# g8a9/multi-modal-emotion

Hardware: AMD Instinct MI355X
Metric: utterances/sec fwd+bwd (+clip_grad_norm_+AdamW inside the timed step), TAV (BERT+Wav2Vec2+VideoMAE) b=32, 1/2/4/8 MI355X (higher is better)
Workload: dtype bf16; 1 GPU; tav_nn.py TAV preset B (bert 12 L + wav2vec2 12 L / 768 + videomae 12 L / 768 on 16 frames + fusion 12 L), global batch 32 = 32 per GPU x 1, text 128 tok, audio 80000 samples, video 16x3x224x224 (104 fusion / 1464 encoder tokens), 547.0 GFLOP forward per utterance; global_batch=32, per_gpu_batch=32, parallelism=dp1, weights=random init (seeded), no checkpoints offline, launch=hipGraph replay

## Files before the change

multi-modal-emotion_amd/csrc/gemm.hip:

```cpp
#include "common.h"
#include <type_traits>
#include "tavhip_internal.h"
#include "gemm_plan.h"

namespace tav {

struct GemmNT {
    const char* A; const char* B; char* C; char* Cpre; const float* bias; const char* gelu_in; const float* resid;
    int M, N, K;
    long lda, ldb, ldc, ld_pre, ld_gelu, ld_resid;
    int nzg;
    long a_zb, a_zg, b_zb, b_zg, c_zb, c_zg, bias_zg;
    long g_zb;
    int act, accumulate;
    float alpha;
    int tiles_m, tiles_n;
    const float* sa; const float* sb;
};

TAV_DEV int swz(int row, int chunk) { return chunk ^ ((row >> 1) & 7); }

enum { NT_GEN = 0, NT_PLAIN = 1, NT_RESID = 2, NT_GELU_D = 3, NT_MUL_D = 4 };
template <typename T, typename TO, int TM, int NST, int NW, int TNW, int EPI = NT_GEN>
__global__ __launch_bounds__(64 * NW, NW == 4 ? 2 : 1) __attribute__((amdgpu_waves_per_eu(2, 2))) void gemm_nt_kernel(const GemmNT p) {
// ... 79 lines not shown
        for (int t = 0; t < TNW; ++t) fb0[t] = *reinterpret_cast<const uint4*>(cB + off_b[0][t]);
#pragma unroll
        for (int t = 0; t < TM; ++t) fa1[t] = *reinterpret_cast<const uint4*>(cA + off_a[1][t]);
#pragma unroll
        for (int t = 0; t < TNW; ++t) fb1[t] = *reinterpret_cast<const uint4*>(cB + off_b[1][t]);
        __builtin_amdgcn_sched_barrier(0);
#pragma unroll
        for (int tn = 0; tn < TNW; ++tn) {
#pragma unroll
            for (int tm = 0; tm < TM; ++tm) {
                if constexpr (F8) mma16_fp8(fb0[tn], fb1[tn], fa0[tm], fa1[tm], acc[tn][tm]);
                else mma16<T>(fb0[tn], fa0[tm], acc[tn][tm]);
            }
            if constexpr (decltype(prefetch)::value) {
                __builtin_amdgcn_sched_barrier(0);
#pragma unroll
                for (int pc = tn * NP / TNW; pc < (tn + 1) * NP / TNW; ++pc) stage_piece(pc, ko, nxt);
                __builtin_amdgcn_sched_barrier(0);
            }
        }
        if constexpr (!F8) {
#pragma unroll
            for (int tn = 0; tn < TNW; ++tn)
#pragma unroll
                for (int tm = 0; tm < TM; ++tm) mma16<T>(fb1[tn], fa1[tm], acc[tn][tm]);
        }
    };
    auto ktile25 = [&](int kt, int cl, int cs, auto issue_s, auto issue_l) {
        constexpr bool IS = decltype(issue_s)::value, IL = decltype(issue_l)::value;
        if constexpr (IS) asm volatile("s_waitcnt vmcnt(%0)" ::"n"(TM) : "memory");
        else wait_vmcnt0();
        __syncthreads();
        const char* cA = sA + cl * TILE_A;
        const char* cB = sB + cs * TILE_B;
        const int nl = cl == 0 ? 2 : cl - 1;
        const int ns = cs ^ 1;
#pragma unroll
        for (int t = 0; t < TM; ++t) fa0[t] = *reinterpret_cast<const uint4*>(cA + off_a[0][t]);
#pragma unroll
        for (int t = 0; t < TNW; ++t) fb0[t] = *reinterpret_cast<const uint4*>(cB + off_b[0][t]);
#pragma unroll
        for (int t = 0; t < TM; ++t) fa1[t] = *reinterpret_cast<const uint4*>(cA + off_a[1][t]);
#pragma unroll
        for (int t = 0; t < TNW; ++t) fb1[t] = *reinterpret_cast<const uint4*>(cB + off_b[1][t]);
        __builtin_amdgcn_sched_barrier(0);
#pragma unroll
        for (int tn = 0; tn < TNW; ++tn) {
#pragma unroll
            for (int tm = 0; tm < TM; ++tm) mma16<T>(fb0[tn], fa0[tm], acc[tn][tm]);
            if constexpr (IS || IL) {
                __builtin_amdgcn_sched_barrier(0);
                if constexpr (IS) {
                    if (tn < PB) stage_b(tn, (unsigned)(kt + 1) * 128u, ns);
                }
                if constexpr (IL) {
                    if (tn >= PB && tn - PB < TM) stage_a(tn - PB, (unsigned)(kt + 2) * 128u, nl);
                }
                __builtin_amdgcn_sched_barrier(0);
            }
        }
#pragma unroll
        for (int tn = 0; tn < TNW; ++tn)
#pragma unroll
            for (int tm = 0; tm < TM; ++tm) mma16<T>(fb1[tn], fa1[tm], acc[tn][tm]);
    };
    if constexpr (R25) {
        static_assert(!R25 || PB + TM <= TNW, "one DMA piece per MFMA group");
        auto stage_l = [&](unsigned ko, int slot) {
#pragma unroll
            for (int j = 0; j < TM; ++j) stage_a(j, ko, slot);
        };
        auto stage_s = [&](unsigned ko, int slot) {
#pragma unroll
            for (int j = 0; j < PB; ++j) stage_b(j, ko, slot);
        };
        stage_l(0u, 0);
        stage_s(0u, 0);
        if (nk > 1) stage_l(128u, 1);
        int cl = 0, cs = 0, kt = 0;
        for (; kt + 2 < nk; ++kt) { ktile25(kt, cl, cs, std::true_type{}, std::true_type{}); cl = cl == 2 ? 0 : cl + 1; cs ^= 1; }
        if (kt + 1 < nk) { ktile25(kt, cl, cs, std::true_type{}, std::false_type{}); cl = cl == 2 ? 0 : cl + 1; cs ^= 1; ++kt; }
        if (kt < nk) ktile25(kt, cl, cs, std::false_type{}, std::false_type{});
    } else {
#pragma unroll
    for (int t = 0; t < NST - 1; ++t)
        if (t < nk) {
#pragma unroll
            for (int pc = 0; pc < NP; ++pc) stage_piece(pc, (unsigned)t * 128u, t);
        }
    int cur = 0;
    int kt = 0;
    for (; kt + NST - 1 < nk; ++kt) { ktile(kt, cur, std::true_type{}); cur = cur + 1 == NST ? 0 : cur + 1; }
    for (; kt < nk; ++kt) { ktile(kt, cur, std::false_type{}); cur = cur + 1 == NST ? 0 : cur + 1; }
    }

    __syncthreads();
    float* sC = reinterpret_cast<float*>(smem);
    constexpr int ROWB_C = BN * 4;
    constexpr int CPR = BN / 4;
    constexpr int LDS_BYTES = NST * (TILE_A + TILE_B);
    constexpr int EP_ROWS = (LDS_BYTES / ROWB_C) < BM ? (LDS_BYTES / ROWB_C) / (16 * TM) * (16 * TM) : BM;
    constexpr int NPASS = BM / EP_ROWS;
    static_assert(EP_ROWS >= 16 * TM && BM % EP_ROWS == 0, "epilogue staging");
    const long coff = zb * p.c_zb + zg * p.c_zg;
    TO* C = reinterpret_cast<TO*>(p.C) + coff;
    TO* Cpre = p.Cpre ? reinterpret_cast<TO*>(p.Cpre) + coff : nullptr;
    const TS* Gin = p.gelu_in ? reinterpret_cast<const TS*>(p.gelu_in) + (zb * p.g_zb + zg * p.c_zg) : nullptr;
    const float alpha = p.alpha * (p.sa ? *p.sa : 1.f) * (p.sb ? *p.sb : 1.f);
    const float* R = p.resid ? p.resid + coff : nullptr;
    constexpr bool GEN = EPI == NT_GEN;
    const bool f_resid = GEN ? (R != nullptr) : (EPI == NT_RESID);
    const bool f_pre = GEN ? (Cpre != nullptr && !(p.act & 2)) : false;
    const bool f_act3 = GEN ? ((p.act & 3) == 3) : (EPI == NT_GELU_D);
    const bool f_gelu = GEN ? ((p.act & 3) == 1) : false;
    const bool f_gin = GEN ? (Gin != nullptr) : (EPI == NT_MUL_D);
    const bool f_gin_d = GEN ? ((p.act & 4) != 0) : true;
    const bool f_acc = GEN ? (p.accumulate != 0) : false;
    const int ch = tid % CPR, rr = tid / CPR;
    constexpr int RPI = 64 * NW / CPR;
    const int n = n0 + 4 * ch;
    f32x4 bv = {0.f, 0.f, 0.f, 0.f};
    if (n < p.N && p.bias) bv = ld4(p.bias + zg * p.bias_zg + n);
    constexpr int NIT = EP_ROWS / RPI;
    static_assert(EP_ROWS % RPI == 0 && NIT <= 16, "epilogue rows per thread");
    const bool interior = m0 + BM <= p.M && n0 + BN <= p.N;
    constexpr int PD = (EPI == NT_MUL_D) ? NIT : (NIT > 8 ? 8 : NIT);
    constexpr bool EARLY = (TNW == 4);
    const bool pre_r = f_resid, pre_g = !pre_r && f_gin && sizeof(TS) == 2, pre_c = !pre_r && !pre_g && f_acc && sizeof(TO) == 4;
    const bool any_side = pre_r || pre_c || pre_g;
    char* const Cb = reinterpret_cast<char*>(C + (long)m0 * p.ldc);
    char* const Pb = Cpre ? reinterpret_cast<char*>(Cpre + (long)m0 * p.ld_pre) : nullptr;
    const char* const Gb = Gin ? reinterpret_cast<const char*>(Gin + (long)m0 * p.ld_gelu) : nullptr;
    const char* const Rb = R ? reinterpret_cast<const char*>(R + (long)m0 * p.ld_resid) : nullptr;
    const unsigned s_c = RPI * (unsigned)p.ldc * sizeof(TO), s_p = RPI * (unsigned)p.ld_pre * sizeof(TO);
    const unsigned s_g = RPI * (unsigned)p.ld_gelu * sizeof(TS), s_r = RPI * (unsigned)p.ld_resid * 4u;
    auto run_pass = [&](int row_lo, auto full_tag) __attribute__((always_inline)) {
        constexpr bool FULL = decltype(full_tag)::value;
        const unsigned row = (unsigned)(row_lo + rr);
        const unsigned o_c = (row * (unsigned)p.ldc + (unsigned)n) * (unsigned)sizeof(TO), o_p = (row * (unsigned)p.ld_pre + (unsigned)n) * (unsigned)sizeof(TO);
        const unsigned o_g = (row * (unsigned)p.ld_gelu + (unsigned)n) * (unsigned)sizeof(TS), o_r = (row * (unsigned)p.ld_resid + (unsigned)n) * 4u;
        f32x4 side[PD];
        auto side_load = [&](int it) __attribute__((always_inline)) -> f32x4 {
            const int m = m0 + row_lo + rr + it * RPI;
            f32x4 v = {0.f, 0.f, 0.f, 0.f};
            if (FULL || (n < p.N && m < p.M)) {
                if (pre_r) v = ld4(reinterpret_cast<const float*>(Rb + (o_r + it * s_r)));
                else if (pre_c) { if constexpr (sizeof(TO) == 4) v = ld4(reinterpret_cast<const float*>(Cb + (o_c + it * s_c))); }
                else if (pre_g) {
                    const uint2 w = *reinterpret_cast<const uint2*>(Gb + (o_g + it * s_g));
                    v[0] = __uint_as_float(w.x);
                    v[1] = __uint_as_float(w.y);
                }
            }
            return v;
        };
        auto side_loads = [&]() __attribute__((always_inline)) {
            if (!any_side) return;
#pragma unroll
            for (int it = 0; it < PD; ++it) side[it] = side_load(it);
        };
        if constexpr (EARLY) side_loads();
        if (wm * 16 * TM >= row_lo && wm * 16 * TM < row_lo + EP_ROWS) {
#pragma unroll
            for (int tm = 0; tm < TM; ++tm) {
                const int r = wm * 16 * TM + tm * 16 + i - row_lo;
#pragma unroll
                for (int tn = 0; tn < TNW; ++tn) {
                    const int cc = wn * 4 * TNW + tn * 4 + g;
                    *reinterpret_cast<f32x4*>(reinterpret_cast<char*>(sC) + r * ROWB_C + ((cc ^ (r & 31)) << 4)) = acc[tn][tm];
                }
            }
        }
        if constexpr (!EARLY) side_loads();
        __syncthreads();
        if (FULL || n < p.N) {
            auto staged = [&](int it) __attribute__((always_inline)) -> f32x4 {
                const int r = rr + it * RPI;
                return *reinterpret_cast<const f32x4*>(reinterpret_cast<const char*>(sC) + r * ROWB_C + ((ch ^ (r & 31)) << 4));
            };
            f32x4 v_next = staged(0);
#pragma unroll
            for (int it = 0; it < NIT; ++it) {
                const int r = rr + it * RPI;
                const int m = m0 + row_lo + r;
                const f32x4 sv = side[it % PD];
                if constexpr (PD < NIT) { if (it + PD < NIT && any_side) side[it % PD] = side_load(it + PD); }
                f32x4 v = v_next;
                if (it + 1 < NIT) v_next = staged(it + 1);
                if (FULL || m < p.M) {
                    v = v * alpha + bv;
                    if (f_pre) st4(reinterpret_cast<TO*>(Pb + (o_p + it * s_p)), v);
                    if (f_act3) {
                        f32x4 d, y4;
                        gelu_both4_t<TS>(v, y4, d);
                        v = y4;
                        if (GEN ? Cpre != nullptr : true) st4(reinterpret_cast<TO*>(Pb + (o_p + it * s_p)), d);
                    } else if (f_gelu) { v[0] = gelu_t<TS>(v[0]); v[1] = gelu_t<TS>(v[1]); v[2] = gelu_t<TS>(v[2]); v[3] = gelu_t<TS>(v[3]); }
                    if (f_gin) {
                        f32x4 u;
                        if (pre_g) {
                            const uint32_t w0 = __float_as_uint(sv[0]), w1 = __float_as_uint(sv[1]);
                            u = f32x4{bf16_bits_to_f32(w0 & 0xffffu), bf16_bits_to_f32(w0 >> 16), bf16_bits_to_f32(w1 & 0xffffu), bf16_bits_to_f32(w1 >> 16)};
                        }
                        else u = ld4(reinterpret_cast<const TS*>(Gb + (o_g + it * s_g)));
                        if (f_gin_d) v *= u;
                        else { v[0] *= gelu_grad_t<TS>(u[0]); v[1] *= gelu_grad_t<TS>(u[1]); v[2] *= gelu_grad_t<TS>(u[2]); v[3] *= gelu_grad_t<TS>(u[3]); }
                    }
                    if (pre_r) v += sv;
                    if (f_acc) {
                        if (pre_c) v += sv;
                        else v += ld4(reinterpret_cast<const TO*>(Cb + (o_c + it * s_c)));
                    }
                    st4(reinterpret_cast<TO*>(Cb + (o_c + it * s_c)), v);
                }
            }
        }
    };
    if constexpr (GEN) {
#pragma unroll 1
        for (int pass = 0; pass < NPASS; ++pass) {
            if (pass) __syncthreads();
            run_pass(pass * EP_ROWS, std::false_type{});
        }
    } else {
        if (interior) {
#pragma unroll
            for (int pass = 0; pass < NPASS; ++pass) {
                if (pass) __syncthreads();
                run_pass(pass * EP_ROWS, std::true_type{});
            }
        } else {
#pragma unroll
            for (int pass = 0; pass < NPASS; ++pass) {
                if (pass) __syncthreads();
                run_pass(pass * EP_ROWS, std::false_type{});
            }
        }
    }
}

struct GemmTN {
    const char* A; const char* B; float* S;
    float* bias_part;
    int bias_spread;
    int N1, N2;
    long lda, ldb;
    int rows_per_batch;
    long a_zb, b_zb;
    int chunk_rows;
    int chunks_per_batch;
    int tiles_1, tiles_2;
};

template <typename T> struct TNTile {
    static constexpr int ES = ET<T>::ES, ROWB = 128 * ES, CPR = ROWB / 16;
    static TAV_DEV int sw(int row, int chunk) { return ES == 2 ? (chunk ^ ((row & 7) << 1)) : (chunk ^ (((row >> 2) & 1) << 2)); }
};
template <typename T> TAV_DEV uint4 tn_frag(const char* tile, int krow0, int col0, int lane);
template <> TAV_DEV uint4 tn_frag<bf16>(const char* tile, int krow0, int col0, int lane) {
    using TT = TNTile<bf16>;
    const int g = lane >> 4, i = lane & 15, q = i >> 2, p = i & 3;
    const int r0 = krow0 + 4 * g + q, r1 = r0 + 16;
    const int cb = (col0 + 4 * p) * 2;
    const char* a0 = tile + r0 * TT::ROWB + (TT::sw(r0, cb >> 4) << 4) + (cb & 15);
    const char* a1 = tile + r1 * TT::ROWB + (TT::sw(r1, cb >> 4) << 4) + (cb & 15);
    const uint2 lo = lds_read_tr16(a0), hi = lds_read_tr16(a1);
    return make_uint4(lo.x, lo.y, hi.x, hi.y);
}
template <> TAV_DEV uint4 tn_frag<float>(const char* tile, int krow0, int col0, int lane) {
    using TT = TNTile<float>;
    const int g = lane >> 4, i = lane & 15;
    const int cb = (col0 + i) * 4;
    uint4 r;
    uint32_t* rr = reinterpret_cast<uint32_t*>(&r);
#pragma unroll
    for (int t = 0; t < 4; ++t) {
        const int row = krow0 + 4 * g + t;
        rr[t] = *reinterpret_cast<const uint32_t*>(tile + row * TT::ROWB + (TT::sw(row, cb >> 4) << 4) + (cb & 15));
    }
    return r;
}

template <typename T> TAV_DEV uint4 ones_frag();
template <> TAV_DEV uint4 ones_frag<bf16>() { return make_uint4(0x3f803f80u, 0x3f803f80u, 0x3f803f80u, 0x3f803f80u); }
template <> TAV_DEV uint4 ones_frag<float>() { return make_uint4(0x3f800000u, 0x3f800000u, 0x3f800000u, 0x3f800000u); }

template <typename T> struct TNShape { static constexpr int KT = 64, NST = 2; };

template <typename T>
TAV_DEV void gemm_tn_body(const GemmTN& p, const int tile, const int split) {
    using TT = TNTile<T>;
    constexpr int ES = ET<T>::ES, PK = ET<T>::PK, KSTEP = ET<T>::KSTEP;
    constexpr int BT = 128, KT = TNShape<T>::KT, NST = TNShape<T>::NST;
    constexpr int ROWB = TT::ROWB, CPR = TT::CPR;
    constexpr int TILE_BYTES = KT * ROWB;
    constexpr int RPI = 64 / CPR;
    constexpr int WROWS = KT / 4;
    constexpr int NINST = WROWS / RPI;
    static_assert(KT % KSTEP == 0 && WROWS % RPI == 0 && NINST >= 1, "TN tile shape");
    extern __shared__ __attribute__((aligned(16))) char smem[];
    char* sA = smem;
    char* sB = smem + NST * TILE_BYTES;

    const int tid = threadIdx.x, lane = tid & 63, wave = tid >> 6;
    const int g = lane >> 4, i = lane & 15;
    const int w1 = wave >> 1, w2 = wave & 1;

    int t1, t2;
    if (p.tiles_1 >= p.tiles_2) { t1 = tile / p.tiles_2; t2 = tile - t1 * p.tiles_2; }
    else { t2 = tile / p.tiles_1; t1 = tile - t2 * p.tiles_1; }
    const int n1_0 = t1 * BT, n2_0 = t2 * BT;
    const int zb = split / p.chunks_per_batch, ck = split - zb * p.chunks_per_batch;
    const int row_begin = ck * p.chunk_rows;
    int row_end = row_begin + p.chunk_rows; row_end = row_end < p.rows_per_batch ? row_end : p.rows_per_batch;

    const char* Ab = p.A + zb * p.a_zb * ES;
    const char* Bb = p.B + zb * p.b_zb * ES;

    const int lrow = lane / CPR, lslot = lane % CPR;
    const int a_cmax = (p.N1 - n1_0) * ES / 16, b_cmax = (p.N2 - n2_0) * ES / 16;

    f32x4 acc[4][4];
#pragma unroll
    for (int a = 0; a < 4; ++a)
#pragma unroll
        for (int b = 0; b < 4; ++b) acc[a][b] = f32x4{0.f, 0.f, 0.f, 0.f};
    const bool do_bias = p.bias_part != nullptr && (p.bias_spread || t2 == 0);
    const int bias_mod = p.bias_spread ? p.tiles_2 : 1, bias_rem = p.bias_spread ? t2 : 0;
    f32x4 bacc[2] = {f32x4{0.f, 0.f, 0.f, 0.f}, f32x4{0.f, 0.f, 0.f, 0.f}};
    const uint4 ones = ones_frag<T>();

    const int nrows = row_end - row_begin;
    const int nk = (nrows + KT - 1) / KT;
    const unsigned ldsA = __builtin_amdgcn_readfirstlane(lds_addr(sA) + wave * WROWS * ROWB);
    const unsigned ldsB = __builtin_amdgcn_readfirstlane(lds_addr(sB) + wave * WROWS * ROWB);
    const char* Ab0 = Ab + ((long)row_begin * p.lda + n1_0) * ES;
    const char* Bb0 = Bb + ((long)row_begin * p.ldb + n2_0) * ES;
    unsigned offA[NINST], offB[NINST];
#pragma unroll
    for (int j = 0; j < NINST; ++j) {
        const int trow = wave * WROWS + j * RPI + lrow;
        int ca = TT::sw(trow, lslot); ca = ca < a_cmax ? ca : 0;
        int cb = TT::sw(trow, lslot); cb = cb < b_cmax ? cb : 0;
        offA[j] = (unsigned)(trow * p.lda * ES + ca * 16);
        offB[j] = (unsigned)(trow * p.ldb * ES + cb * 16);
    }
    const unsigned strideA = (unsigned)(KT * p.lda * ES), strideB = (unsigned)(KT * p.ldb * ES);
    auto stage = [&](int kt, int buf) {
        const int base_row = row_begin + kt * KT + wave * WROWS;
        const bool full = (kt + 1) * KT <= nrows;
        if (full) {
            const unsigned ka = kt * strideA, kb = kt * strideB;
#pragma unroll
            for (int j = 0; j < NINST; ++j) {
                glds16_m0(Ab0 + ka, offA[j], ldsA + buf * TILE_BYTES + j * 1024);
                glds16_m0(Bb0 + kb, offB[j], ldsB + buf * TILE_BYTES + j * 1024);
            }
        } else {
#pragma unroll 1
            for (int j = 0; j < NINST; ++j) {
                const int r = j * RPI + lrow;
                const int trow = wave * WROWS + r;
                const int ca = TT::sw(trow, lslot), cb = TT::sw(trow, lslot);
                const bool ok = (kt * KT + trow) < nrows;
                uint4 va = make_uint4(0, 0, 0, 0), vb = va;
                if (ok && ca < a_cmax) va = *reinterpret_cast<const uint4*>(Ab + ((long)(base_row + r) * p.lda + n1_0) * ES + ca * 16);
                if (ok && cb < b_cmax) vb = *reinterpret_cast<const uint4*>(Bb + ((long)(base_row + r) * p.ldb + n2_0) * ES + cb * 16);
                *reinterpret_cast<uint4*>(sA + buf * TILE_BYTES + trow * ROWB + lslot * 16) = va;
                *reinterpret_cast<uint4*>(sB + buf * TILE_BYTES + trow * ROWB + lslot * 16) = vb;
            }
        }
    };
    auto compute = [&](int cur, int kt_now) {
        const char* cA = sA + cur * TILE_BYTES;
        const char* cB = sB + cur * TILE_BYTES;
        const bool bias_now = do_bias && (kt_now % bias_mod) == bias_rem;
#pragma unroll
        for (int s = 0; s < KT / KSTEP; ++s) {
            uint4 f1[4], f2[4];
#pragma unroll
            for (int t = 0; t < 4; ++t) {
                f1[t] = tn_frag<T>(cA, s * KSTEP, w1 * 64 + t * 16, lane);
                f2[t] = tn_frag<T>(cB, s * KSTEP, w2 * 64 + t * 16, lane);
            }
#pragma unroll
            for (int a = 0; a < 4; ++a)
#pragma unroll
                for (int b = 0; b < 4; ++b) mma16<T>(f2[b], f1[a], acc[a][b]);
            if (bias_now) {
                if (w2 == 0) { mma16<T>(ones, f1[0], bacc[0]); mma16<T>(ones, f1[1], bacc[1]); }
                else { mma16<T>(ones, f1[2], bacc[0]); mma16<T>(ones, f1[3], bacc[1]); }
            }
        }
    };

#pragma unroll
    for (int t = 0; t < NST - 1; ++t)
        if (t < nk) stage(t, t);
    int cur = 0, kt = 0;
    for (; kt + NST - 1 < nk; ++kt) {
        asm volatile("s_waitcnt vmcnt(%0)" ::"n"((NST - 2) * 2 * NINST) : "memory");
        __syncthreads();
        stage(kt + NST - 1, cur == 0 ? NST - 1 : cur - 1);
        compute(cur, kt);
        cur = cur + 1 == NST ? 0 : cur + 1;
    }
    for (; kt < nk; ++kt) {
        wait_vmcnt0();
        __syncthreads();
        compute(cur, kt);
        cur = cur + 1 == NST ? 0 : cur + 1;
    }
    __syncthreads();

    if (do_bias && g == 0) {
        const long slot = p.bias_spread ? (long)split * p.tiles_2 + t2 : split;
#pragma unroll
        for (int j = 0; j < 2; ++j) {
            const int n1 = n1_0 + w1 * 64 + (2 * w2 + j) * 16 + i;
            if (n1 < p.N1) p.bias_part[slot * p.N1 + n1] = bacc[j][0];
        }
    }
    float* S = p.S + (long)split * p.N1 * p.N2;
#pragma unroll
    for (int a = 0; a < 4; ++a) {
        const int n1 = n1_0 + w1 * 64 + a * 16 + i;
        if (n1 >= p.N1) continue;
#pragma unroll
        for (int b = 0; b < 4; ++b) {
            const int n2 = n2_0 + w2 * 64 + b * 16 + 4 * g;
            if (n2 >= p.N2) continue;
            st4(S + (long)n1 * p.N2 + n2, acc[a][b]);
        }
    }
}

template <typename T>
__global__ __launch_bounds__(256, 2) void gemm_tn_kernel(const GemmTN p) {
    gemm_tn_body<T>(p, xcd_remap(blockIdx.x, p.tiles_1 * p.tiles_2), blockIdx.y);
}

constexpr int TN_GROUP_MAX = 4;
struct GemmTNGroup {
    GemmTN p[TN_GROUP_MAX];
    int tile_end[TN_GROUP_MAX];
    int n;
};
template <typename T>
__global__ __launch_bounds__(256, 2) void gemm_tn_grouped_kernel(const GemmTNGroup grp) {
    const int t = xcd_remap(blockIdx.x, grp.tile_end[grp.n - 1]);
    int g = 0;
#pragma unroll
    for (int k = 0; k < TN_GROUP_MAX - 1; ++k) g += (k < grp.n - 1 && t >= grp.tile_end[k]) ? 1 : 0;
    const int first = g == 0 ? 0 : grp.tile_end[g - 1];
    gemm_tn_body<T>(grp.p[g], t - first, 0);
}

template <typename T>
TAV_DEV void gemm_tn_big_body(const GemmTN& p, const int tile, const int split) {
    using TT = TNTile<T>;
    static_assert(ET<T>::ES == 2, "bf16 only");
    constexpr int ES = 2, KSTEP = ET<T>::KSTEP, KT = 64, ROWB = TT::ROWB;
    constexpr int SUB = KT * ROWB;
    constexpr int STAGE = 4 * SUB;
    extern __shared__ __attribute__((aligned(16))) char smem[];

    const int tid = threadIdx.x, lane = tid & 63, wave = tid >> 6;
    const int g = lane >> 4, i = lane & 15;
    const int w1 = wave >> 1, w2 = wave & 1;

    int t1, t2;
    if (p.tiles_1 >= p.tiles_2) { t1 = tile / p.tiles_2; t2 = tile - t1 * p.tiles_2; }
    else { t2 = tile / p.tiles_1; t1 = tile - t2 * p.tiles_1; }
    const int n1_0 = t1 * 256, n2_0 = t2 * 256;
    const int row_begin = split * p.chunk_rows;
    int row_end = row_begin + p.chunk_rows; row_end = row_end < p.rows_per_batch ? row_end : p.rows_per_batch;
    const int nrows = row_end - row_begin;
    const int nk = nrows > 0 ? (nrows + KT - 1) / KT : 0;

    const int lrow = lane >> 4, lslot = lane & 15;
    const int a_cmax = (p.N1 - n1_0) * ES / 16, b_cmax = (p.N2 - n2_0) * ES / 16;
    const char* Ab0 = p.A + ((long)row_begin * p.lda + n1_0) * ES;
    const char* Bb0 = p.B + ((long)row_begin * p.ldb + n2_0) * ES;
    unsigned offA[2][2], offB[2][2];
#pragma unroll
    for (int h = 0; h < 2; ++h)
#pragma unroll
        for (int j = 0; j < 2; ++j) {
            const int trow = wave * 8 + j * 4 + lrow;
            int ca = 16 * h + TT::sw(trow, lslot); ca = ca < a_cmax ? ca : 0;
            int cb = 16 * h + TT::sw(trow, lslot); cb = cb < b_cmax ? cb : 0;
            offA[h][j] = (unsigned)(trow * p.lda * ES + ca * 16);
            offB[h][j] = (unsigned)(trow * p.ldb * ES + cb * 16);
        }
    const unsigned strideA = (unsigned)(KT * p.lda * ES), strideB = (unsigned)(KT * p.ldb * ES);
    const unsigned lds0 = __builtin_amdgcn_readfirstlane(lds_addr(smem) + wave * 8 * ROWB);
    constexpr int NSA = 3;
    constexpr int IMG = 2 * SUB;
    constexpr int OFF_B = NSA * IMG;
    auto stage_ragged = [&](int kt, int slot, bool is_b) {
#pragma unroll 1
        for (int e = 0; e < 4; ++e) {
            const int h = e >> 1, j = e & 1;
            const int trow = wave * 8 + j * 4 + lrow;
            const int c = 16 * h + TT::sw(trow, lslot);
            const bool ok = (kt * KT + trow) < nrows;
            const long grow = (long)row_begin + kt * KT + trow;
            uint4 v = make_uint4(0, 0, 0, 0);
            if (!is_b) { if (ok && c < a_cmax) v = *reinterpret_cast<const uint4*>(p.A + (grow * p.lda + n1_0) * ES + c * 16); }
            else { if (ok && c < b_cmax) v = *reinterpret_cast<const uint4*>(p.B + (grow * p.ldb + n2_0) * ES + c * 16); }
            *reinterpret_cast<uint4*>(smem + (is_b ? OFF_B : 0) + slot * IMG + h * SUB + trow * ROWB + lslot * 16) = v;
        }
    };
    auto piece_a = [&](int pc, unsigned ka, int slot) { glds16_m0(Ab0 + ka, offA[pc >> 1][pc & 1], lds0 + slot * IMG + (pc >> 1) * SUB + (pc & 1) * 1024); };
    auto piece_b = [&](int pc, unsigned kb, int slot) { glds16_m0(Bb0 + kb, offB[pc >> 1][pc & 1], lds0 + OFF_B + slot * IMG + (pc >> 1) * SUB + (pc & 1) * 1024); };
    const bool last_ragged = nk > 0 && nk * KT > nrows;
    auto is_dma = [&](int kt) { return kt < nk && !(last_ragged && kt == nk - 1); };
    auto stage_a = [&](int kt, int slot) {
        if (is_dma(kt)) {
#pragma unroll
            for (int pc = 0; pc < 4; ++pc) piece_a(pc, (unsigned)kt * strideA, slot);
        } else stage_ragged(kt, slot, false);
    };
    auto stage_b = [&](int kt, int slot) {
        if (is_dma(kt)) {
#pragma unroll
            for (int pc = 0; pc < 4; ++pc) piece_b(pc, (unsigned)kt * strideB, slot);
        } else stage_ragged(kt, slot, true);
    };

    f32x4 acc[4][8];
#pragma unroll
    for (int a = 0; a < 4; ++a)
#pragma unroll
        for (int b = 0; b < 8; ++b) acc[a][b] = f32x4{0.f, 0.f, 0.f, 0.f};
    const bool do_bias = p.bias_part != nullptr && (p.bias_spread || t2 == 0);
    const int bias_mod = p.bias_spread ? p.tiles_2 : 1, bias_rem = p.bias_spread ? t2 : 0;
    f32x4 bacc[2] = {f32x4{0.f, 0.f, 0.f, 0.f}, f32x4{0.f, 0.f, 0.f, 0.f}};
    const uint4 ones = ones_frag<T>();

    constexpr int AHEAD_A = 2;
    if (nk > 0) { stage_a(0, 0); stage_b(0, 0); if (nk > 1) stage_a(1, 1); }
    int ca = 0;
    for (int kt = 0; kt < nk; ++kt) {
        const int cb = kt & 1;
        if (is_dma(kt + 1)) asm volatile("s_waitcnt vmcnt(4)" ::: "memory");
        else wait_vmcnt0();
        __syncthreads();
        const int na = ca == 0 ? 2 : ca - 1, nb = cb ^ 1;
        const bool dma_b = is_dma(kt + 1), dma_a = is_dma(kt + AHEAD_A);
        if (kt + 1 < nk && !dma_b) stage_b(kt + 1, nb);
        if (kt + AHEAD_A < nk && !dma_a) stage_a(kt + AHEAD_A, na);
        const unsigned ka = (unsigned)(kt + AHEAD_A) * strideA, kb = (unsigned)(kt + 1) * strideB;
        const char* cA = smem + ca * IMG + (w1 >> 1) * SUB;
        const char* cB = smem + OFF_B + cb * IMG + w2 * SUB;
        const bool bias_now = do_bias && (kt % bias_mod) == bias_rem;
#pragma unroll
        for (int s2 = 0; s2 < KT / KSTEP; ++s2) {
            uint4 f1[4], f2[8];
#pragma unroll
            for (int t = 0; t < 4; ++t) f1[t] = tn_frag<T>(cA, s2 * KSTEP, (w1 & 1) * 64 + t * 16, lane);
#pragma unroll
            for (int t = 0; t < 8; ++t) f2[t] = tn_frag<T>(cB, s2 * KSTEP, t * 16, lane);
            __builtin_amdgcn_sched_barrier(0);
#pragma unroll
            for (int b = 0; b < 8; ++b) {
#pragma unroll
                for (int a = 0; a < 4; ++a) mma16<T>(f2[b], f1[a], acc[a][b]);
                if (s2 == 0) {
                    __builtin_amdgcn_sched_barrier(0);
                    if (b < 4) { if (dma_b) piece_b(b, kb, nb); }
                    else { if (dma_a) piece_a(b - 4, ka, na); }
                    __builtin_amdgcn_sched_barrier(0);
                }
            }
            if (bias_now) {
                if (w2 == 0) { mma16<T>(ones, f1[0], bacc[0]); mma16<T>(ones, f1[1], bacc[1]); }
                else { mma16<T>(ones, f1[2], bacc[0]); mma16<T>(ones, f1[3], bacc[1]); }
            }
        }
        ca = ca == 2 ? 0 : ca + 1;
    }
    __syncthreads();

    if (do_bias && g == 0) {
        const long slot = p.bias_spread ? (long)split * p.tiles_2 + t2 : split;
#pragma unroll
        for (int j = 0; j < 2; ++j) {
            const int n1 = n1_0 + w1 * 64 + (2 * w2 + j) * 16 + i;
            if (n1 < p.N1) p.bias_part[slot * p.N1 + n1] = bacc[j][0];
        }
    }
    float* S = p.S + (long)split * p.N1 * p.N2;
#pragma unroll
    for (int a = 0; a < 4; ++a) {
        const int n1 = n1_0 + w1 * 64 + a * 16 + i;
        if (n1 >= p.N1) continue;
#pragma unroll
        for (int b = 0; b < 8; ++b) {
            const int n2 = n2_0 + w2 * 128 + b * 16 + 4 * g;
            if (n2 >= p.N2) continue;
            st4(S + (long)n1 * p.N2 + n2, acc[a][b]);
        }
    }
}

template <typename T>
__global__ __launch_bounds__(512, 1) __attribute__((amdgpu_waves_per_eu(2, 2))) void gemm_tn_grouped_big_kernel(const GemmTNGroup grp) {
    const int t = xcd_remap(blockIdx.x, grp.tile_end[grp.n - 1]);
    int g = 0;
#pragma unroll
    for (int k = 0; k < TN_GROUP_MAX - 1; ++k) g += (k < grp.n - 1 && t >= grp.tile_end[k]) ? 1 : 0;
    const int first = g == 0 ? 0 : grp.tile_end[g - 1];
    gemm_tn_big_body<T>(grp.p[g], t - first, blockIdx.y);
}

struct TNGroupReduce {
    const float* slabs[TN_GROUP_MAX]; float* out[TN_GROUP_MAX]; const float* bias_part[TN_GROUP_MAX]; float* dbias[TN_GROUP_MAX];
    long n4[TN_GROUP_MAX];
    long end4[TN_GROUP_MAX];
    int N1[TN_GROUP_MAX];
    int nbias[TN_GROUP_MAX];
    int n, nsplit;
};
__global__ void tn_group_reduce_kernel(const TNGroupReduce r) {
    const long gid = (long)blockIdx.x * blockDim.x + threadIdx.x;
    if (gid >= r.end4[r.n - 1]) return;
    int k = 0;
#pragma unroll
    for (int q = 0; q < TN_GROUP_MAX - 1; ++q) k += (q < r.n - 1 && gid >= r.end4[q]) ? 1 : 0;
    const long local = gid - (k == 0 ? 0 : r.end4[k - 1]);
    const float* S = r.slabs[k];
    f32x4 v = {0.f, 0.f, 0.f, 0.f};
    for (int s2 = 0; s2 < r.nsplit; ++s2) v += ld4(S + ((long)s2 * r.n4[k] + local) * 4);
    st4(r.out[k] + local * 4, v);
    if (r.dbias[k] && local < r.N1[k]) {
        float b = 0.f;
        for (int s2 = 0; s2 < r.nbias[k]; ++s2) b += r.bias_part[k][(long)s2 * r.N1[k] + local];
        r.dbias[k][local] = b;
    }
}
__global__ void tn_group_bias_reduce_kernel(const TNGroupReduce r, int total_n1) {
    int gid = blockIdx.x * blockDim.x + threadIdx.x;
    if (gid >= total_n1) return;
    int k = 0;
    while (k < r.n - 1 && gid >= r.N1[k]) { gid -= r.N1[k]; ++k; }
    if (!r.dbias[k]) return;
    float b = 0.f;
    for (int s2 = 0; s2 < r.nbias[k]; ++s2) b += r.bias_part[k][(long)s2 * r.N1[k] + gid];
    r.dbias[k][gid] = b;
}

__global__ void splitk_reduce_kernel(const float* __restrict__ S, float* __restrict__ out, int nsplit, long n_elems, int N2,
                                     int inner, int outer, int accumulate, float scale, const float* __restrict__ bias_part,
                                     float* __restrict__ dbias, int N1) {
    const long gid = (long)blockIdx.x * blockDim.x + threadIdx.x;
    if (dbias && gid < N1) {
        float b = 0.f;
        for (int s = 0; s < nsplit; ++s) b += bias_part[(long)s * N1 + gid];
        b *= scale;
        dbias[gid] = accumulate ? dbias[gid] + b : b;
    }
    const long idx4 = gid * 4;
    if (idx4 >= n_elems) return;
    f32x4 v = {0.f, 0.f, 0.f, 0.f};
    for (int s = 0; s < nsplit; ++s) v += ld4(S + (long)s * n_elems + idx4);
    v *= scale;
    if (outer == 1) {
        if (accumulate) v += ld4(out + idx4);
        st4(out + idx4, v);
    } else {
        const long n1 = idx4 / N2; const int n2 = (int)(idx4 - n1 * N2);
#pragma unroll
        for (int e = 0; e < 4; ++e) {
            const int q = n2 + e;
            const long o = n1 * N2 + (long)(q % inner) * outer + q / inner;
            out[o] = accumulate ? out[o] + v[e] : v[e];
        }
    }
}

__global__ void bias_reduce_kernel(const float* __restrict__ part, float* __restrict__ out, int nsplit, int N1, int accumulate, float scale) {
    const int n = blockIdx.x * blockDim.x + threadIdx.x;
    if (n >= N1) return;
    float s = 0.f;
    for (int k = 0; k < nsplit; ++k) s += part[(long)k * N1 + n];
    s *= scale;
    out[n] = accumulate ? out[n] + s : s;
}

template <typename T>
__global__ void colsum_partial_kernel(const T* __restrict__ X, float* __restrict__ part, int M, int N, long ld, int rows_per_block) {
    const int n = blockIdx.x * blockDim.x + threadIdx.x;
    const int r_begin = blockIdx.y * rows_per_block;
    int r_end = r_begin + rows_per_block; r_end = r_end < M ? r_end : M;
    if (n >= N) return;
    float s0 = 0.f, s1 = 0.f, s2 = 0.f, s3 = 0.f;
    int r = r_begin;
    for (; r + 3 < r_end; r += 4) {
        s0 += ET<T>::ld(X + (long)r * ld + n); s1 += ET<T>::ld(X + (long)(r + 1) * ld + n);
        s2 += ET<T>::ld(X + (long)(r + 2) * ld + n); s3 += ET<T>::ld(X + (long)(r + 3) * ld + n);
    }
    for (; r < r_end; ++r) s0 += ET<T>::ld(X + (long)r * ld + n);
    part[(long)blockIdx.y * N + n] = (s0 + s1) + (s2 + s3);
}
__global__ void colsum_final_kernel(const float* __restrict__ part, float* __restrict__ out, int nparts, int N, int accumulate) {
    const int n = blockIdx.x * blockDim.x + threadIdx.x;
    if (n >= N) return;
    float s0 = 0.f, s1 = 0.f, s2 = 0.f, s3 = 0.f;
    int k = 0;
    for (; k + 3 < nparts; k += 4) {
        s0 += part[(long)k * N + n]; s1 += part[(long)(k + 1) * N + n]; s2 += part[(long)(k + 2) * N + n]; s3 += part[(long)(k + 3) * N + n];
    }
    for (; k < nparts; ++k) s0 += part[(long)k * N + n];
    const float s = (s0 + s1) + (s2 + s3);
    out[n] = accumulate ? out[n] + s : s;
}

}

using namespace tav;

static_assert(NT_GEN == plan::EPI_GEN && NT_PLAIN == plan::EPI_PLAIN && NT_RESID == plan::EPI_RESID && NT_GELU_D == plan::EPI_GELU_D &&
              NT_MUL_D == plan::EPI_MUL_D && TN_GROUP_MAX == plan::TN_PROBLEMS_MAX, "gemm_plan.h mirrors these");

template <int DTYPE> struct NtElem;
template <> struct NtElem<TAV_F32> { using type = float; };
template <> struct NtElem<TAV_BF16> { using type = bf16; };
template <> struct NtElem<TAV_FP8> { using type = fp8; };
using NtKernel = void (*)(const GemmNT);
#define TAV_NT_KERNEL(IN, OUT, TM, NST, NW, TNW, EPI) gemm_nt_kernel<NtElem<TAV_##IN>::type, NtElem<TAV_##OUT>::type, TM, NST, NW, TNW, NT_##EPI>,
static const NtKernel nt_kernels[] = {TAV_NT_KERNELS(TAV_NT_KERNEL)};
#undef TAV_NT_KERNEL
static_assert(sizeof(nt_kernels) / sizeof(nt_kernels[0]) == plan::nt_num_keys, "one kernel per key");

extern "C" int tav_gemm_nt_schedule(const tav_gemm_nt_args* a, int32_t* tile, int32_t* rows_first, int32_t* tile_rest) {
    if (!tile || !rows_first || !tile_rest) return TAV_ERR_NULL;
    const int rc = plan::nt_validate(a, false);
    if (rc != 0) return rc;
    int tm, rb, tr;
    plan::nt_plan(a, &tm, &rb, &tr);
    *tile = tm; *rows_first = rb; *tile_rest = rb < a->M ? tr : 0;
    return 0;
}

static int nt_enqueue(const tav_gemm_nt_args* a, GemmNT p, int tm, hipStream_t stream) {
    const plan::NtLaunch L = plan::nt_launch(a, p.M, tm);
    const int k = plan::nt_key_index(L.key);
    if (k < 0) return TAV_ERR_DTYPE;
    p.tiles_m = L.tiles_m; p.tiles_n = L.tiles_n;
    hipLaunchKernelGGL(nt_kernels[k], dim3(L.grid_x, L.grid_y), dim3(L.block), L.lds, stream, p);
    return 0;
}

extern "C" int tav_gemm_nt(const tav_gemm_nt_args* a, void* stream_) {
    hipStream_t stream = (hipStream_t)stream_;
    { const int rc = plan::nt_validate(a, true); if (rc != 0) return rc; }
    GemmNT p;
    p.A = (const char*)a->A; p.B = (const char*)a->B; p.C = (char*)a->C; p.Cpre = (char*)a->C_pre; p.bias = a->bias;
    p.gelu_in = (const char*)a->gelu_in; p.resid = a->resid;
    p.M = (int)a->M; p.N = (int)a->N; p.K = (int)a->K;
    p.lda = a->lda; p.ldb = a->ldb; p.ldc = a->ldc; p.ld_pre = a->ld_pre; p.ld_gelu = a->ld_gelu_in; p.ld_resid = a->ld_resid;
    p.nzg = a->nzg > 0 ? a->nzg : 1;
    p.a_zb = a->a_zb; p.a_zg = a->a_zg; p.b_zb = a->b_zb; p.b_zg = a->b_zg; p.c_zb = a->c_zb; p.c_zg = a->c_zg; p.bias_zg = a->bias_zg;
    p.g_zb = a->gelu_zb ? a->gelu_zb : a->c_zb;
    p.act = a->act; p.accumulate = a->accumulate; p.alpha = a->alpha;
    p.sa = a->in_dtype == TAV_FP8 ? a->a_dequant : nullptr; p.sb = a->in_dtype == TAV_FP8 ? a->b_dequant : nullptr;
    int tm, rows_big, tm_rest;
    plan::nt_plan(a, &tm, &rows_big, &tm_rest);
    if (rows_big < p.M) {
        const plan::NtSplit s = plan::nt_split(a, rows_big);
        GemmNT q = p;
        q.M = s.M_rest;
        q.A = p.A + s.a_bytes; q.C = p.C + s.c_bytes;
        if (p.Cpre) q.Cpre = p.Cpre + s.pre_bytes;
        if (p.gelu_in) q.gelu_in = p.gelu_in + s.gelu_bytes;
        if (p.resid) q.resid = p.resid + s.resid_elems;
        p.M = rows_big;
        int rc = nt_enqueue(a, p, 16, stream);
        if (rc == 0) rc = nt_enqueue(a, q, tm_rest, stream);
        if (rc != 0) return rc;
    } else {
        const int rc = nt_enqueue(a, p, tm, stream);
        if (rc != 0) return rc;
    }
    return (int)hipGetLastError();
}

extern "C" int tav_gemm_tn_splits(int64_t n1, int64_t n2, int64_t rows_per_batch, int64_t nbatch, int32_t* chunk_rows, int32_t* nsplit) {
    if (!chunk_rows || !nsplit || n1 <= 0 || n2 <= 0 || rows_per_batch <= 0 || nbatch <= 0) return TAV_ERR_SHAPE;
    plan::tn_splits(n1, n2, rows_per_batch, nbatch, chunk_rows, nsplit);
    return 0;
}

static void tn_group_fill(const tav_gemm_tn_problem* probs, int nprob, long rows, const plan::TnGroupPlan& P, const plan::TnGroupLayout& L,
                          bool use_ws, float* ws, GemmTNGroup* grp, TNGroupReduce* red) {
    for (int k = 0; k < TN_GROUP_MAX; ++k) {
        const tav_gemm_tn_problem& a = probs[k < nprob ? k : nprob - 1];
        float* const bias_ws = L.bias_off[k] >= 0 ? ws + L.bias_off[k] : nullptr;
        GemmTN& p = grp->p[k];
        p.A = (const char*)a.A; p.B = (const char*)a.B; p.N1 = (int)a.N1; p.N2 = (int)a.N2; p.lda = a.lda; p.ldb = a.ldb;
        p.rows_per_batch = (int)rows; p.a_zb = 0; p.b_zb = 0; p.chunk_rows = (int)P.chunk; p.chunks_per_batch = P.nsplit;
        p.tiles_1 = L.tiles_1[k]; p.tiles_2 = L.tiles_2[k];
        p.S = L.slab_off[k] >= 0 ? ws + L.slab_off[k] : a.out;
        p.bias_part = use_ws ? bias_ws : a.dbias; p.bias_spread = use_ws ? 1 : 0;
        grp->tile_end[k] = L.tile_end[k];
        red->slabs[k] = p.S; red->out[k] = a.out; red->dbias[k] = a.dbias; red->N1[k] = (int)a.N1; red->n4[k] = L.n4[k];
        red->nbias[k] = L.nbias[k]; red->bias_part[k] = bias_ws; red->end4[k] = L.end4[k];
    }
    grp->n = nprob; red->n = nprob; red->nsplit = P.nsplit;
}

extern "C" int tav_gemm_tn_grouped(const tav_gemm_tn_problem* probs, int32_t nprob, int64_t rows, int32_t dtype, void* stream_) {
    hipStream_t stream = (hipStream_t)stream_;
    if (!probs) return TAV_ERR_NULL;
    if (nprob <= 0 || nprob > TN_GROUP_MAX || rows <= 0) return TAV_ERR_SHAPE;
    if (dtype != TAV_BF16 && dtype != TAV_F32) return TAV_ERR_DTYPE;
    { const int rc = plan::tn_validate_group(probs, nprob, rows, dtype); if (rc != 0) return rc; }
    const plan::TnGroupPlan P = plan::tn_plain_plan(rows);
    const plan::TnGroupLayout L = plan::tn_group_layout(probs, nprob, P, false);
    GemmTNGroup grp;
    TNGroupReduce red;
    tn_group_fill(probs, nprob, rows, P, L, false, nullptr, &grp, &red);
    dim3 grid(L.total), block(256);
    if (dtype == TAV_BF16) hipLaunchKernelGGL((gemm_tn_grouped_kernel<bf16>), grid, block, 4 * 64 * 256, stream, grp);
    else hipLaunchKernelGGL((gemm_tn_grouped_kernel<float>), grid, block, 4 * 64 * 512, stream, grp);
    return (int)hipGetLastError();
}

extern "C" int64_t tav_gemm_tn_grouped_ws_bytes(const tav_gemm_tn_problem* probs, int32_t nprob, int64_t rows, int32_t dtype, int32_t flags) {
    if (!probs || nprob <= 0 || nprob > TN_GROUP_MAX || rows <= 0) return 0;
    return plan::tn_big_plan(probs, nprob, rows, dtype, flags).ws_floats * 4;
}

extern "C" int tav_gemm_tn_grouped_ws(const tav_gemm_tn_problem* probs, int32_t nprob, int64_t rows, int32_t dtype, void* workspace,
                                      int64_t workspace_bytes, int32_t flags, void* stream_) {
    hipStream_t stream = (hipStream_t)stream_;
    if (!probs) return TAV_ERR_NULL;
    if (nprob <= 0 || nprob > TN_GROUP_MAX || rows <= 0) return TAV_ERR_SHAPE;
    if (dtype != TAV_BF16 && dtype != TAV_F32) return TAV_ERR_DTYPE;
    const plan::TnGroupPlan P = plan::tn_big_plan(probs, nprob, rows, dtype, flags);
    if (P.ws_floats > 0 && (!workspace || workspace_bytes < P.ws_floats * 4)) return tav_gemm_tn_grouped(probs, nprob, rows, dtype, stream_);
    if (plan::tn_has_empty_split(P, rows)) return TAV_ERR_SHAPE;
    { const int rc = plan::tn_validate_group(probs, nprob, rows, dtype); if (rc != 0) return rc; }
    const plan::TnGroupLayout L = plan::tn_group_layout(probs, nprob, P, true);
    GemmTNGroup grp;
    TNGroupReduce red;
    tn_group_fill(probs, nprob, rows, P, L, true, (float*)workspace, &grp, &red);
    if (P.big) hipLaunchKernelGGL((gemm_tn_grouped_big_kernel<bf16>), dim3(L.total, P.nsplit), dim3(512), 5 * 2 * 64 * 256, stream, grp);
    else if (dtype == TAV_BF16) hipLaunchKernelGGL((gemm_tn_grouped_kernel<bf16>), dim3(L.total), dim3(256), 4 * 64 * 256, stream, grp);
    else hipLaunchKernelGGL((gemm_tn_grouped_kernel<float>), dim3(L.total), dim3(256), 4 * 64 * 512, stream, grp);
    if (P.nsplit > 1) hipLaunchKernelGGL(tn_group_reduce_kernel, dim3((unsigned)((L.end4[TN_GROUP_MAX - 1] + 255) / 256)), dim3(256), 0, stream, red);
    else if (L.any_bias) hipLaunchKernelGGL(tn_group_bias_reduce_kernel, dim3((unsigned)((L.total_n1 + 255) / 256)), dim3(256), 0, stream, red, L.total_n1);
    return (int)hipGetLastError();
}

extern "C" int tav_gemm_tn(const tav_gemm_tn_args* a, void* stream_) {
    hipStream_t stream = (hipStream_t)stream_;
    if (!a || !a->slabs) return TAV_ERR_NULL;
    { const int rc = plan::tn_validate_problem(a->A, a->B, a->out, a->N1, a->N2, a->lda, a->ldb, a->a_zb, a->b_zb, a->rows_per_batch, a->nbatch, a->dtype);
      if (rc != 0) return rc; }
    if (a->chunk_rows <= 0 || a->chunk_rows % 64) return TAV_ERR_SHAPE;
    GemmTN p;
    p.A = (const char*)a->A; p.B = (const char*)a->B; p.S = a->slabs;
    p.bias_part = a->dbias ? a->bias_partials : nullptr; p.bias_spread = 0;
    if (a->dbias && !a->bias_partials) return TAV_ERR_NULL;
    p.N1 = (int)a->N1; p.N2 = (int)a->N2; p.lda = a->lda; p.ldb = a->ldb;
    p.rows_per_batch = (int)a->rows_per_batch; p.a_zb = a->a_zb; p.b_zb = a->b_zb;
    p.chunk_rows = a->chunk_rows;
    p.chunks_per_batch = (int)((a->rows_per_batch + a->chunk_rows - 1) / a->chunk_rows);
    const int nsplit = p.chunks_per_batch * (int)a->nbatch;
    if (nsplit != a->nsplit) return TAV_ERR_SHAPE;
    p.tiles_1 = (p.N1 + 127) / 128; p.tiles_2 = (p.N2 + 127) / 128;
    const int inner = a->perm_inner > 0 ? a->perm_inner : p.N2, outer = a->perm_outer > 0 ? a->perm_outer : 1;
    if (outer > 1 && inner * outer != p.N2) return TAV_ERR_SHAPE;
    dim3 grid(p.tiles_1 * p.tiles_2, nsplit), block(256);
    if (a->dtype == TAV_BF16) {
        const size_t lds = 4 * 64 * 256;
        hipLaunchKernelGGL((gemm_tn_kernel<bf16>), grid, block, lds, stream, p);
    } else {
        const size_t lds = 4 * 64 * 512;
        hipLaunchKernelGGL((gemm_tn_kernel<float>), grid, block, lds, stream, p);
    }
    int e = (int)hipGetLastError();
    if (e) return e;
// ... 21 lines not shown
```

Before: 424.2 utterances/s.

## Peel ragged k-tiles out of TN GEMM main loops and software-pipeline fragment loads

Splits the TN weight-gradient GEMM K-loops into a steady-state part that always issues async global-to-LDS copies and a peeled tail that handles the ragged last tile. The per-iteration full/ragged and DMA checks become compile-time specialisations. In the big-tile kernel, the second k-step's LDS fragments are loaded while the first k-step's MFMAs run, and the wave index is made uniform via readfirstlane. Bias-slot selection uses a counter instead of a modulo. The intent is to cut branch and scalar overhead and hide LDS latency, at the cost of more registers and code size, which could hurt occupancy.

```diff
diff --git a/multi-modal-emotion_amd/csrc/gemm.hip b/multi-modal-emotion_amd/csrc/gemm.hip
--- a/multi-modal-emotion_amd/csrc/gemm.hip
+++ b/multi-modal-emotion_amd/csrc/gemm.hip
@@ -405,7 +405,7 @@
     char* sA = smem;
     char* sB = smem + NST * TILE_BYTES;
 
-    const int tid = threadIdx.x, lane = tid & 63, wave = tid >> 6;
+    const int tid = threadIdx.x, lane = tid & 63, wave = __builtin_amdgcn_readfirstlane(tid >> 6);
     const int g = lane >> 4, i = lane & 15;
     const int w1 = wave >> 1, w2 = wave & 1;
 
@@ -450,68 +450,83 @@
     }
     const unsigned strideA = (unsigned)(KT * p.lda * ES), strideB = (unsigned)(KT * p.ldb * ES);
     auto stage = [&](int kt, int buf) {
+        const unsigned ka = kt * strideA, kb = kt * strideB;
+#pragma unroll
+        for (int j = 0; j < NINST; ++j) {
+            glds16_m0(Ab0 + ka, offA[j], ldsA + buf * TILE_BYTES + j * 1024);
+            glds16_m0(Bb0 + kb, offB[j], ldsB + buf * TILE_BYTES + j * 1024);
+        }
+    };
+    auto stage_ragged = [&](int kt, int buf) {
         const int base_row = row_begin + kt * KT + wave * WROWS;
-        const bool full = (kt + 1) * KT <= nrows;
-        if (full) {
-            const unsigned ka = kt * strideA, kb = kt * strideB;
-#pragma unroll
-            for (int j = 0; j < NINST; ++j) {
-                glds16_m0(Ab0 + ka, offA[j], ldsA + buf * TILE_BYTES + j * 1024);
-                glds16_m0(Bb0 + kb, offB[j], ldsB + buf * TILE_BYTES + j * 1024);
-            }
-        } else {
 #pragma unroll 1
-            for (int j = 0; j < NINST; ++j) {
-                const int r = j * RPI + lrow;
-                const int trow = wave * WROWS + r;
-                const int ca = TT::sw(trow, lslot), cb = TT::sw(trow, lslot);
-                const bool ok = (kt * KT + trow) < nrows;
-                uint4 va = make_uint4(0, 0, 0, 0), vb = va;
-                if (ok && ca < a_cmax) va = *reinterpret_cast<const uint4*>(Ab + ((long)(base_row + r) * p.lda + n1_0) * ES + ca * 16);
-                if (ok && cb < b_cmax) vb = *reinterpret_cast<const uint4*>(Bb + ((long)(base_row + r) * p.ldb + n2_0) * ES + cb * 16);
-                *reinterpret_cast<uint4*>(sA + buf * TILE_BYTES + trow * ROWB + lslot * 16) = va;
-                *reinterpret_cast<uint4*>(sB + buf * TILE_BYTES + trow * ROWB + lslot * 16) = vb;
-            }
+        for (int j = 0; j < NINST; ++j) {
+            const int r = j * RPI + lrow;
+            const int trow = wave * WROWS + r;
+            const int ca = TT::sw(trow, lslot), cb = TT::sw(trow, lslot);
+            const bool ok = (kt * KT + trow) < nrows;
+            uint4 va = make_uint4(0, 0, 0, 0), vb = va;
+            if (ok && ca < a_cmax) va = *reinterpret_cast<const uint4*>(Ab + ((long)(base_row + r) * p.lda + n1_0) * ES + ca * 16);
+            if (ok && cb < b_cmax) vb = *reinterpret_cast<const uint4*>(Bb + ((long)(base_row + r) * p.ldb + n2_0) * ES + cb * 16);
+            *reinterpret_cast<uint4*>(sA + buf * TILE_BYTES + trow * ROWB + lslot * 16) = va;
+            *reinterpret_cast<uint4*>(sB + buf * TILE_BYTES + trow * ROWB + lslot * 16) = vb;
         }
     };
-    auto compute = [&](int cur, int kt_now) {
+    int bias_cnt = bias_rem;
+    auto compute = [&](int cur) {
         const char* cA = sA + cur * TILE_BYTES;
         const char* cB = sB + cur * TILE_BYTES;
-        const bool bias_now = do_bias && (kt_now % bias_mod) == bias_rem;
-#pragma unroll
-        for (int s = 0; s < KT / KSTEP; ++s) {
-            uint4 f1[4], f2[4];
-#pragma unroll
-            for (int t = 0; t < 4; ++t) {
-                f1[t] = tn_frag<T>(cA, s * KSTEP, w1 * 64 + t * 16, lane);
-                f2[t] = tn_frag<T>(cB, s * KSTEP, w2 * 64 + t * 16, lane);
+        const bool bias_now = do_bias && bias_cnt == 0;
+        bias_cnt = bias_cnt == 0 ? bias_mod - 1 : bias_cnt - 1;
+        constexpr int NS = KT / KSTEP, G = ES == 2 ? NS : 1;
+#pragma unroll
+        for (int s0 = 0; s0 < NS; s0 += G) {
+            uint4 f1[G][4], f2[G][4];
+#pragma unroll
+            for (int s = 0; s < G; ++s)
+#pragma unroll
+                for (int t = 0; t < 4; ++t) {
+                    f1[s][t] = tn_frag<T>(cA, (s0 + s) * KSTEP, w1 * 64 + t * 16, lane);
+                    f2[s][t] = tn_frag<T>(cB, (s0 + s) * KSTEP, w2 * 64 + t * 16, lane);
+                }
+#pragma unroll
+            for (int s = 0; s < G; ++s) {
+#pragma unroll
+                for (int a = 0; a < 4; ++a)
+#pragma unroll
+                    for (int b = 0; b < 4; ++b) mma16<T>(f2[s][b], f1[s][a], acc[a][b]);
+                if (bias_now) {
+                    if (w2 == 0) { mma16<T>(ones, f1[s][0], bacc[0]); mma16<T>(ones, f1[s][1], bacc[1]); }
+                    else { mma16<T>(ones, f1[s][2], bacc[0]); mma16<T>(ones, f1[s][3], bacc[1]); }
+                }
             }
-#pragma unroll
-            for (int a = 0; a < 4; ++a)
-#pragma unroll
-                for (int b = 0; b < 4; ++b) mma16<T>(f2[b], f1[a], acc[a][b]);
-            if (bias_now) {
-                if (w2 == 0) { mma16<T>(ones, f1[0], bacc[0]); mma16<T>(ones, f1[1], bacc[1]); }
-                else { mma16<T>(ones, f1[2], bacc[0]); mma16<T>(ones, f1[3], bacc[1]); }
-            }
         }
     };
 
+    const int nd = nrows / KT;
 #pragma unroll
     for (int t = 0; t < NST - 1; ++t)
-        if (t < nk) stage(t, t);
+        if (t < nk) { if (t < nd) stage(t, t); else stage_ragged(t, t); }
     int cur = 0, kt = 0;
-    for (; kt + NST - 1 < nk; ++kt) {
+    for (; kt + NST - 1 < nd; ++kt) {
         asm volatile("s_waitcnt vmcnt(%0)" ::"n"((NST - 2) * 2 * NINST) : "memory");
         __syncthreads();
         stage(kt + NST - 1, cur == 0 ? NST - 1 : cur - 1);
-        compute(cur, kt);
+        compute(cur);
         cur = cur + 1 == NST ? 0 : cur + 1;
+    }
+    if (kt + NST - 1 < nk) {
+        asm volatile("s_waitcnt vmcnt(%0)" ::"n"((NST - 2) * 2 * NINST) : "memory");
+        __syncthreads();
+        stage_ragged(kt + NST - 1, cur == 0 ? NST - 1 : cur - 1);
+        compute(cur);
+        cur = cur + 1 == NST ? 0 : cur + 1;
+        ++kt;
     }
     for (; kt < nk; ++kt) {
         wait_vmcnt0();
         __syncthreads();
-        compute(cur, kt);
+        compute(cur);
         cur = cur + 1 == NST ? 0 : cur + 1;
     }
     __syncthreads();
@@ -568,7 +583,7 @@
     constexpr int STAGE = 4 * SUB;
     extern __shared__ __attribute__((aligned(16))) char smem[];
 
-    const int tid = threadIdx.x, lane = tid & 63, wave = tid >> 6;
+    const int tid = threadIdx.x, lane = tid & 63, wave = __builtin_amdgcn_readfirstlane(tid >> 6);
     const int g = lane >> 4, i = lane & 15;
     const int w1 = wave >> 1, w2 = wave & 1;
 
@@ -642,48 +657,63 @@
     f32x4 bacc[2] = {f32x4{0.f, 0.f, 0.f, 0.f}, f32x4{0.f, 0.f, 0.f, 0.f}};
     const uint4 ones = ones_frag<T>();
 
-    constexpr int AHEAD_A = 2;
-    if (nk > 0) { stage_a(0, 0); stage_b(0, 0); if (nk > 1) stage_a(1, 1); }
-    int ca = 0;
-    for (int kt = 0; kt < nk; ++kt) {
-        const int cb = kt & 1;
-        if (is_dma(kt + 1)) asm volatile("s_waitcnt vmcnt(4)" ::: "memory");
+    int ca = 0, cb = 0, bias_cnt = bias_rem;
+    auto ktile = [&](int kt, auto issue_b, auto issue_a, auto tail) {
+        constexpr bool IB = decltype(issue_b)::value, IA = decltype(issue_a)::value, TAIL = decltype(tail)::value;
+        if constexpr (IB) asm volatile("s_waitcnt vmcnt(4)" ::: "memory");
         else wait_vmcnt0();
         __syncthreads();
         const int na = ca == 0 ? 2 : ca - 1, nb = cb ^ 1;
-        const bool dma_b = is_dma(kt + 1), dma_a = is_dma(kt + AHEAD_A);
-        if (kt + 1 < nk && !dma_b) stage_b(kt + 1, nb);
-        if (kt + AHEAD_A < nk && !dma_a) stage_a(kt + AHEAD_A, na);
-        const unsigned ka = (unsigned)(kt + AHEAD_A) * strideA, kb = (unsigned)(kt + 1) * strideB;
+        if constexpr (TAIL) {
+            if (last_ragged && kt + 1 == nk - 1) stage_ragged(kt + 1, nb, true);
+            if (last_ragged && kt + 2 == nk - 1) stage_ragged(kt + 2, na, false);
+        }
+        const unsigned ka = (unsigned)(kt + 2) * strideA, kb = (unsigned)(kt + 1) * strideB;
         const char* cA = smem + ca * IMG + (w1 >> 1) * SUB;
         const char* cB = smem + OFF_B + cb * IMG + w2 * SUB;
-        const bool bias_now = do_bias && (kt % bias_mod) == bias_rem;
-#pragma unroll
-        for (int s2 = 0; s2 < KT / KSTEP; ++s2) {
-            uint4 f1[4], f2[8];
-#pragma unroll
-            for (int t = 0; t < 4; ++t) f1[t] = tn_frag<T>(cA, s2 * KSTEP, (w1 & 1) * 64 + t * 16, lane);
-#pragma unroll
-            for (int t = 0; t < 8; ++t) f2[t] = tn_frag<T>(cB, s2 * KSTEP, t * 16, lane);
+        const bool bias_now = do_bias && bias_cnt == 0;
+        uint4 f1[4], f2[8], g1[4];
+#pragma unroll
+        for (int t = 0; t < 4; ++t) f1[t] = tn_frag<T>(cA, 0, (w1 & 1) * 64 + t * 16, lane);
+#pragma unroll
+        for (int t = 0; t < 8; ++t) f2[t] = tn_frag<T>(cB, 0, t * 16, lane);
+        __builtin_amdgcn_sched_barrier(0);
+#pragma unroll
+        for (int b = 0; b < 8; ++b) {
+#pragma unroll
+            for (int a = 0; a < 4; ++a) mma16<T>(f2[b], f1[a], acc[a][b]);
             __builtin_amdgcn_sched_barrier(0);
-#pragma unroll
-            for (int b = 0; b < 8; ++b) {
-#pragma unroll
-                for (int a = 0; a < 4; ++a) mma16<T>(f2[b], f1[a], acc[a][b]);
-                if (s2 == 0) {
-                    __builtin_amdgcn_sched_barrier(0);
-                    if (b < 4) { if (dma_b) piece_b(b, kb, nb); }
-                    else { if (dma_a) piece_a(b - 4, ka, na); }
-                    __builtin_amdgcn_sched_barrier(0);
-                }
+            if constexpr (IB) { if (b < 4) piece_b(b, kb, nb); }
+            if constexpr (IA) { if (b >= 4) piece_a(b - 4, ka, na); }
+            f2[b] = tn_frag<T>(cB, KSTEP, b * 16, lane);
+            if (b == 3) {
+#pragma unroll
+                for (int t = 0; t < 4; ++t) g1[t] = tn_frag<T>(cA, KSTEP, (w1 & 1) * 64 + t * 16, lane);
             }
-            if (bias_now) {
-                if (w2 == 0) { mma16<T>(ones, f1[0], bacc[0]); mma16<T>(ones, f1[1], bacc[1]); }
-                else { mma16<T>(ones, f1[2], bacc[0]); mma16<T>(ones, f1[3], bacc[1]); }
-            }
+            __builtin_amdgcn_sched_barrier(0);
+        }
+        if (bias_now) {
+            if (w2 == 0) { mma16<T>(ones, f1[0], bacc[0]); mma16<T>(ones, f1[1], bacc[1]); }
+            else { mma16<T>(ones, f1[2], bacc[0]); mma16<T>(ones, f1[3], bacc[1]); }
+        }
+#pragma unroll
+        for (int b = 0; b < 8; ++b)
+#pragma unroll
+            for (int a = 0; a < 4; ++a) mma16<T>(f2[b], g1[a], acc[a][b]);
+        if (bias_now) {
+            if (w2 == 0) { mma16<T>(ones, g1[0], bacc[0]); mma16<T>(ones, g1[1], bacc[1]); }
+            else { mma16<T>(ones, g1[2], bacc[0]); mma16<T>(ones, g1[3], bacc[1]); }
         }
         ca = ca == 2 ? 0 : ca + 1;
-    }
+        cb ^= 1;
+        bias_cnt = bias_cnt == 0 ? bias_mod - 1 : bias_cnt - 1;
+    };
+    if (nk > 0) { stage_a(0, 0); stage_b(0, 0); if (nk > 1) stage_a(1, 1); }
+    const int nd = last_ragged ? nk - 1 : nk;
+    int kt = 0;
+    for (; kt + 2 < nd; ++kt) ktile(kt, std::true_type{}, std::true_type{}, std::false_type{});
+    if (kt + 1 < nd) { ktile(kt, std::true_type{}, std::false_type{}, std::true_type{}); ++kt; }
+    for (; kt < nk; ++kt) ktile(kt, std::false_type{}, std::false_type{}, std::true_type{});
     __syncthreads();
 
     if (do_bias && g == 0) {
```

New measurement: 428.5 utterances/s (median of 6 runs). +1.0%, better.
